# yechuan51/huffman

Measured on AMD Instinct MI355X. Metric: encode + decode throughput GB/s and % HBM3E peak, 16 GiB Zipf(1.1), 1/2/4/8 GPU, higher is better.
Workload: dtype u8; 1 GPU; 16 GiB Zipf(1.1) bytes per GPU: hist16 -> codebook -> pack -> decode, one global bit stream; bytes_per_gpu=17179869184, total_bytes=17179869184, symbols_per_gpu=8589934592, parallelism=single, payload_bytes_rank0=12416072164, max_code_len=22

## Files before the change

### huffman_amd/csrc/hz_chain.hip

```cpp
#include <stdio.h>
#include <stdlib.h>

#include "hz_decode_device.h"
#include "hz_walk_device.h"

namespace hz {

constexpr int kChainWalkWaves = 16;
constexpr uint32_t kChainRecs = 256;
constexpr uint32_t kSegRing = 16 + 1;
constexpr uint32_t kRingRow = kChainWalkWaves * 64;

struct ChainBlk {
    unsigned long long b0, b1;
    unsigned long long rec;
    long long out;
    uint32_t lo, hi;
    uint32_t last;
    uint32_t lhl;
};
static_assert(sizeof(ChainBlk) == 48, "ChainBlk");

struct ChainArgs {
    uint64_t nchains, cbits;
// ... 394 lines not shown
}

HZ_DEV void chain_store(const DecArgs& a, const ChainMeta& m, int lane, const uint32_t* pk) {
    uint16_t* out16 = reinterpret_cast<uint16_t*>(a.out);
    const uint32_t lo = m.lhl & 0x1ffu, hi = chain_meta_hi(m), last = m.lhl >> 18;
    const bool full = lo == 0 && hi == kChainRecs && last == 8 && m.out >= 0 &&
                      (uint64_t)m.out + (uint64_t)kBlockSyms <= a.nsym;
    if (full) {
        const long long ob = m.out;
#pragma unroll
        for (int c = 0; c < kChainsPerLane; ++c) {
            uint32_t* q = reinterpret_cast<uint32_t*>(out16 + ob + 8 * (64 * c + lane));
            u32x4a2 v = u32x4a2{pk[4 * c], pk[4 * c + 1], pk[4 * c + 2], pk[4 * c + 3]};
            __builtin_nontemporal_store(v, reinterpret_cast<u32x4a2*>(q));
        }
        return;
    }
#pragma unroll
    for (int c = 0; c < kChainsPerLane; ++c) {
        const uint32_t t = 64u * c + (uint32_t)lane;
        if (t < lo || t >= hi) continue;
        const long long o = m.out + 8ll * t;
        if (o < 0 || (uint64_t)o >= a.nsym) continue;
        uint32_t cn = t + 1 == hi ? last : 8u;
        cn = a.nsym - (uint64_t)o < cn ? (uint32_t)(a.nsym - (uint64_t)o) : cn;
        if (cn == 8) {
            *reinterpret_cast<u32x4a2*>(out16 + o) = u32x4a2{pk[4 * c], pk[4 * c + 1], pk[4 * c + 2], pk[4 * c + 3]};
        } else {
            for (uint32_t q = 0; q < cn; ++q) out16[o + q] = (uint16_t)(pk[4 * c + (q >> 1)] >> (16 * (q & 1)));
        }
    }
}

HZ_DEV void dec_wave_chain(const DecArgs& a, const ChainArgs& y, uint64_t nb, const uint32_t* lds, uint32_t* stg,
                           uint32_t slot, uint64_t b, uint64_t stride, int lane) {
    constexpr int C = 2 * kChainsPerLane;
    const __amdgpu_buffer_rsrc_t l2r = lut_l2_rsrc(a.l2);
    ChainMeta mc[2], mn[2], mn2[2];
    uint4 sc[2][kStageUnroll], sn[2][kStageUnroll];
#pragma unroll
    for (int j = 0; j < 2; ++j) {
        chain_meta_load(y, b + j, nb, mc[j]);
        chain_meta_load(y, b + stride + j, nb, mn[j]);
    }
#pragma unroll
    for (int j = 0; j < 2; ++j) chain_rec_load(y, lane, mc[j]);
    auto as_pipe = [](const ChainMeta& m) { PipeMeta p; p.b0 = m.b0; p.b1 = m.b1; p.sub = 0; return p; };
#pragma unroll
    for (int j = 0; j < 2; ++j) dec_stage_prefetch(a, as_pipe(mc[j]), lane, sc[j]);
    for (; b < nb; b += stride) {
#pragma unroll
        for (int j = 0; j < 2; ++j) chain_rec_load(y, lane, mn[j]);
        uint32_t p1[C];
#pragma unroll
        for (int j = 0; j < 2; ++j) {
            uint64_t w0;
            dec_stage_commit<true>(a, as_pipe(mc[j]), slot >> 2, stg + j * slot, lane, sc[j], w0);
            uint32_t off[kChainsPerLane];
            dec_chain_offsets(chain_meta_sub(mc[j], lane), mc[j].b0, mc[j].b1 - mc[j].b0, lane, off);
            const uint32_t top = (uint32_t)(stg - lds) + (uint32_t)(j + 1) * slot - 1u;
            const uint32_t base = top * 32u - (uint32_t)(mc[j].b0 + a.bit_adj - (w0 << 5));
#pragma unroll
            for (int c = 0; c < kChainsPerLane; ++c) p1[j * kChainsPerLane + c] = base - off[c];
        }
        __builtin_amdgcn_wave_barrier();
        uint32_t pk[2][kSPT / 2];
        PipeLane st[C];
        uint32_t g[C];
        auto finish = [&](int c, int q) {
            const uint32_t ee = st[c].e > g[c] ? st[c].e : g[c];
            p1[c] -= ee >> 24;
            const int i = ((c % kChainsPerLane) * kChainSyms + q) >> 1;
            if (q & 1) pk[c / kChainsPerLane][i] = __builtin_amdgcn_perm(ee, pk[c / kChainsPerLane][i], 0x06050201u);
            else pk[c / kChainsPerLane][i] = ee;
        };
        auto issue4 = [&](int c, int q) {
            __builtin_amdgcn_s_setprio(2);
            dec_pipe_ldsn<4>(a, lds, p1 + c, st + c, 16u * (uint32_t)q);
#pragma unroll
            for (int t = 0; t < 4; ++t)
                g[c + t] = __builtin_amdgcn_raw_buffer_load_b32(l2r, st[c + t].gi, 0, 0);
            __builtin_amdgcn_s_setprio(0);
        };
        issue4(0, 0);
#pragma unroll
        for (int q = 0; q < kChainSyms; ++q) {
            issue4(4, q);
            if (q == kPfStep) {
#pragma unroll
                for (int j = 0; j < 2; ++j) dec_stage_prefetch(a, as_pipe(mn[j]), lane, sn[j]);
#pragma unroll
                for (int j = 0; j < 2; ++j) chain_meta_load(y, b + 2 * stride + j, nb, mn2[j]);
            }
#pragma unroll
            for (int c = 0; c < 4; ++c) finish(c, q);
            if (q + 1 < kChainSyms) issue4(0, q + 1);
#pragma unroll
            for (int c = 4; c < 8; ++c) finish(c, q);
        }
        __builtin_amdgcn_wave_barrier();
#pragma unroll
        for (int j = 0; j < 2; ++j)
            if (b + j < nb) chain_store(a, mc[j], lane, pk[j]);
#pragma unroll
        for (int j = 0; j < 2; ++j) {
            mc[j] = mn[j];
            mn[j] = mn2[j];
#pragma unroll
            for (int u = 0; u < kStageUnroll; ++u) sc[j][u] = sn[j][u];
        }
    }
}

__global__ __launch_bounds__(kDecPipe2Threads) void k_chain_decode(DecArgs a, ChainArgs y) {
    extern __shared__ __attribute__((aligned(16))) uint32_t lds[];
    copy_lds_table(lds, a.lds_img, a.lds_words);
    const int lane = threadIdx.x & 63;
    const uint32_t wid = wave_id();
    typedef const __attribute__((address_space(4))) unsigned long long* cu64p;
    const uint64_t nb = ((cu64p)y.info)[0];
    if (nb == 0) return;
    const uint32_t slot = (uint32_t)__builtin_amdgcn_readfirstlane((int)dec_slot_words(((cu64p)y.info)[1], a.max_len));
    const uint32_t nwave = blockDim.x >> 6;
    uint32_t nw2 = a.region_words / (2 * slot);
    nw2 = nw2 < nwave ? nw2 : nwave;
    if (nw2 == 0) {
        if (threadIdx.x == 0) atomicOr(a.err, 128u);
        return;
    }
    if (wid >= nw2) return;
    const uint64_t b = 2 * ((uint64_t)blockIdx.x * nw2 + wid), stride = 2 * (uint64_t)gridDim.x * nw2;
    dec_wave_chain(a, y, nb, lds, lds + a.lds_words + wid * 2 * slot, slot, b, stride, lane);
}

__global__ __launch_bounds__(kSyncThreads) void k_chain_decode_serial(DecArgs a, ChainArgs y) {
    extern __shared__ __attribute__((aligned(16))) uint32_t lds[];
    copy_lds_table(lds, a.lds_img, a.lds_words);
    uint16_t* out16 = reinterpret_cast<uint16_t*>(a.out);
    const uint64_t nrec = y.info[0] * kChainRecs;
    const uint64_t stride = (uint64_t)gridDim.x * blockDim.x;
    for (uint64_t i = (uint64_t)blockIdx.x * blockDim.x + threadIdx.x; i < nrec; i += stride) {
        const ChainBlk& d = y.blk[i / kChainRecs];
        const uint32_t t = (uint32_t)(i % kChainRecs);
        if (t < d.lo || t >= d.hi) continue;
        const long long o = d.out + 8ll * t;
        const uint32_t cn = t + 1 == d.hi ? d.last : 8u;
        BitReader r;
        br_init(r, a, d.b0 + (uint16_t)(y.rec[d.rec + t] - (uint16_t)d.b0) + a.bit_adj);
        for (uint32_t q = 0; q < cn; ++q) {
            uint32_t sym;
            const uint32_t L = br_next<DEC_LUT>(r, a, lds, sym);
            if (L == 0) { atomicOr(a.err, 2u); break; }
            if (o + q >= 0 && (uint64_t)(o + q) < a.nsym) out16[o + q] = (uint16_t)sym;
        }
    }
}

template <int MODE>
__global__ __launch_bounds__(kSyncThreads) void k_chain_tail(DecArgs a, ChainArgs y) {
    extern __shared__ __attribute__((aligned(16))) uint32_t lds[];
    copy_lds_table(lds, a.lds_img, a.lds_words);
    uint16_t* out16 = reinterpret_cast<uint16_t*>(a.out);
    const uint64_t stride = (uint64_t)gridDim.x * blockDim.x;
    const uint64_t last = a.nsym - 1;
    for (uint64_t c = (uint64_t)blockIdx.x * blockDim.x + threadIdx.x; c < y.nchains; c += stride) {
// ... 255 lines not shown
        const bool deep = t.dec_max_len > t.chain_esc_m;
        const void* fn = deep ? (const void*)k_chain_walk<true> : (const void*)k_chain_walk<false>;
        if ((e = ensure_lds_limit(fn, (int)(kChainWalkWaves * 64 * (kSegRing * 4 + 16)))) != hipSuccess) return e;
        const uint64_t wgs = (g.nchains + threads - 1) / threads;
        if (deep) hipLaunchKernelGGL(k_chain_walk<true>, dim3(wgs), dim3(threads), ring_bytes, s, w, y);
        else hipLaunchKernelGGL(k_chain_walk<false>, dim3(wgs), dim3(threads), ring_bytes, s, w, y);
        cap_check(s, "walk");
    }
    if ((e = chain_fix_and_meta(st, t, ncu, s)) != hipSuccess) return e;
    st->valid = true;
    return hipSuccess;
}

hipError_t chain_refix(ChainState* st, const Tables& t, uint64_t entry0, int ncu, hipStream_t s) {
    if (!st->valid) return hipErrorInvalidValue;
    st->y.entry0 = entry0 != ~0ull ? entry0 - st->base : entry0;
    return chain_fix_and_meta(st, t, ncu, s);
}

hipError_t chain_decode(ChainState* st, const Tables& t, uint64_t nsym, uint8_t* d_out, unsigned long long* d_end,
                        int ncu, hipStream_t s) {
    if (!st->valid) return hipErrorInvalidValue;
    DecArgs d = st->d;
    const ChainArgs& y = st->y;
    d.out = d_out;
    d.nsym = nsym;
    hipError_t e;
    if ((e = hipMemsetAsync(y.info + 2, 0xff, 8, s)) != hipSuccess) return e;
    if (nsym && !chain_pipelined(t)) {
        if ((e = ensure_lds_limit((const void*)k_chain_decode_serial, kLdsBytes)) != hipSuccess) return e;
        hipLaunchKernelGGL(k_chain_decode_serial, dim3(4 * ncu), dim3(kSyncThreads), t.chain_lds_bytes, s, d, y);
    }
    if (nsym && chain_pipelined(t)) {
        if ((e = ensure_lds_limit((const void*)k_chain_decode, kLdsBytes)) != hipSuccess) return e;
        const uint64_t bits = st->g.pend - st->g.pbeg;
        uint64_t avg = (uint64_t)(chain_avg(t, bits, nsym) * kBlockSyms);
        avg = avg < (uint64_t)kBlockSyms * (uint32_t)d.max_len ? avg : (uint64_t)kBlockSyms * (uint32_t)d.max_len;
        const uint32_t worst = dec_slot_words_max(d.max_len);
        uint32_t est = dec_slot_words(avg + avg / 16 + 256, d.max_len);
        est = est < worst ? est : worst;
        const uint32_t table = d.lds_words;
        if (table < kDecMinLdsWords || table + worst > kLdsBytes / 4) return hipErrorInvalidValue;
        uint32_t nslot = (kLdsBytes / 4 - table) / est;
        nslot = nslot > 2 * kDecPipe2Threads / 64 ? 2 * kDecPipe2Threads / 64 : nslot;
        nslot &= ~1u;
        DecArgs b = d;
        b.region_words = nslot * est;
        if (b.region_words < 2 * worst && table + 2 * worst <= kLdsBytes / 4) b.region_words = 2 * worst;
        const int threads = 64 * (int)((nslot / 2) ? nslot / 2 : 1);
        const uint32_t lds = 4 * (table + b.region_words);
        hipLaunchKernelGGL(k_chain_decode, dim3(ncu), dim3(threads), lds, s, b, y);
        cap_check(s, "decode");
    }
    if (nsym) {
        if ((e = ensure_lds_limit((const void*)k_chain_tail<DEC_LUT>, kLdsBytes)) != hipSuccess) return e;
        const uint64_t wgs = grid_clamp((y.nchains + kSyncThreads - 1) / kSyncThreads, (uint64_t)ncu);
        hipLaunchKernelGGL(k_chain_tail<DEC_LUT>, dim3(wgs), dim3(kSyncThreads), t.chain_lds_bytes, s, d, y);
    }
    if (d_end) {
        if (st->base == 0) {
            if ((e = hipMemcpyAsync(d_end, y.info + 2, 8, hipMemcpyDeviceToDevice, s)) != hipSuccess) return e;
        } else {
            hipLaunchKernelGGL(k_chain_end, dim3(1), dim3(64), 0, s, (const unsigned long long*)y.info, d_end, st->base);
        }
    }
    cap_check(s, "tail+end");
    return hipGetLastError();
}

}
```

### huffman_amd/csrc/hz_decode.hip

```cpp
#include <stdlib.h>

#include <type_traits>

#include "hz_decode_device.h"

namespace hz {


template <bool WIDE>
HZ_DEV void dec_stage(const DecArgs& a, uint64_t b0, uint64_t b1, uint32_t npc_max, uint32_t* stg, int lane,
                      uint64_t& w0) {
    w0 = ((b0 >> 5) & ~3ull) - 4;
    const uint64_t wend = (b1 >> 5) + (WIDE ? 3 : 2);
    uint32_t npc = (uint32_t)((wend - w0 + 3) >> 2);
    npc = npc < npc_max ? npc : npc_max;
    uint4 v[kStageUnroll];
#pragma unroll
    for (int u = 0; u < kStageUnroll; ++u) {
        const uint32_t p = (uint32_t)lane + (uint32_t)u * kWave;
        if (p < npc) v[u] = dec_stage_load(a, w0 + 4ull * p);
    }
#pragma unroll
    for (int u = 0; u < kStageUnroll; ++u) {
        const uint32_t p = (uint32_t)lane + (uint32_t)u * kWave;
        if (p < npc)
            reinterpret_cast<uint4*>(stg)[p] = make_uint4(bswap32(v[u].x), bswap32(v[u].y), bswap32(v[u].z), bswap32(v[u].w));
    }
    for (uint32_t p = (uint32_t)lane + kStageUnroll * kWave; p < npc; p += kWave) {
        const uint4 x = dec_stage_load(a, w0 + 4ull * p);
        reinterpret_cast<uint4*>(stg)[p] = make_uint4(bswap32(x.x), bswap32(x.y), bswap32(x.z), bswap32(x.w));
    }
}

// ... 195 lines not shown
            const uint32_t sym = lut_leaf_sym(ee);
            const int i = (c * kChainSyms + q) >> 1;
            if (q & 1) pk[i] |= sym << 16;
            else pk[i] = sym;
        };
        auto issue2 = [&](int c) {
            dec_pipe_lds2(a, lds, stg, pos[c], pos[c + 1], st[c], st[c + 1]);
            g[c] = l2g[st[c].gi];
            g[c + 1] = l2g[st[c + 1].gi];
        };
        issue2(0);
#pragma unroll
        for (int q = 0; q < kChainSyms; ++q) {
            issue2(2);
            if (q == kPfStep) {
                dec_stage_prefetch(a, mn, lane, sn);
                dec_meta_load(a, b + 2 * stride, lane, mn2);
            }
            finish(0, q);
            finish(1, q);
            if (q + 1 < kChainSyms) issue2(0);
            finish(2, q);
            finish(3, q);
        }
        __builtin_amdgcn_wave_barrier();
        dec_store(a, b, lane, pk);
        mc = mn;
        mn = mn2;
#pragma unroll
        for (int u = 0; u < kStageUnroll; ++u) sc[u] = sn[u];
    }
}

template <int NS, typename A>
HZ_DEV void dec_wave_pipe2(const A& a, const uint32_t* lds, uint32_t* stg, uint32_t slot, uint64_t b,
                           uint64_t stride, int lane) {
    constexpr int C = 2 * kChainsPerLane;
    constexpr int H = kChainSyms / 2;
    static_assert(kChainsPerLane == 4, "four pairs of chains over two blocks");
    static_assert(kChainSyms == 8 && kPfStep == H, "a block's prefetch issues at the top of its second half");
    const __amdgpu_buffer_rsrc_t l2r = lut_l2_rsrc(a.l2);
    PipeMeta mn[2], mn2;
    uint4 sn[NS];
    uint32_t p1[C];
    uint32_t pk[2][kSPT / 2];
    PipeLane st[C];
    uint32_t g[C];
    auto commit = [&](int j) {
        uint64_t w0;
        dec_stage_commit<true>(a, mn[j], slot >> 2, stg + j * slot, lane, sn, w0);
        uint32_t off[kChainsPerLane];
        dec_chain_offsets(mn[j].sub, mn[j].b0, mn[j].b1 - mn[j].b0, lane, off);
        const uint32_t top = (uint32_t)(stg - lds) + (uint32_t)(j + 1) * slot - 1u;
        const uint32_t base = top * 32u - (uint32_t)(mn[j].b0 + a.bit_adj - (w0 << 5));
#pragma unroll
        for (int c = 0; c < kChainsPerLane; ++c) p1[j * kChainsPerLane + c] = base - off[c];
        mn[j] = mn2;
    };
    auto prefetch = [&](int j, uint64_t after) {
        dec_stage_prefetch(a, mn[j], lane, sn);
        dec_meta_load(a, after, lane, mn2);
    };
    auto finish = [&](int c, int q) {
        const uint32_t ee = st[c].e > g[c] ? st[c].e : g[c];
        p1[c] -= ee >> 24;
        const int i = ((c % kChainsPerLane) * kChainSyms + q) >> 1;
        if (q & 1) pk[c / kChainsPerLane][i] = __builtin_amdgcn_perm(ee, pk[c / kChainsPerLane][i], 0x06050201u);
        else pk[c / kChainsPerLane][i] = ee;
    };
    auto issue4 = [&](int c, int q) {
        __builtin_amdgcn_s_setprio(2);
        dec_pipe_ldsn<4>(a, lds, p1 + c, st + c, 16u * (uint32_t)q);
#pragma unroll
        for (int t = 0; t < 4; ++t)
            g[c + t] = __builtin_amdgcn_raw_buffer_load_b32(l2r, st[c + t].gi, 0, 0);
        __builtin_amdgcn_s_setprio(0);
    };
    auto finish4 = [&](int c, int q) {
#pragma unroll
        for (int t = 0; t < 4; ++t) finish(c + t, q);
    };
    if (b >= a.nblocks) return;
    dec_meta_load(a, b, lane, mn[0]);
    dec_meta_load(a, b + 1, lane, mn[1]);
    prefetch(0, b + stride);
    commit(0);
    prefetch(1, b + 1 + stride);
    commit(1);
    __builtin_amdgcn_wave_barrier();
    issue4(0, 0);
#pragma unroll
    for (int q = 0; q < H; ++q) {
        finish4(0, q);
        issue4(0, q + 1);
    }
    for (; b < a.nblocks; b += stride) {
#pragma unroll
        for (int t = 0; t < H; ++t) {
            issue4(4, t);
            if (t == 0) prefetch(0, b + 2 * stride);
            finish4(0, H + t);
            if (t + 1 < H) {
                issue4(0, H + t + 1);
            } else {
                __builtin_amdgcn_wave_barrier();
                dec_store(a, b, lane, pk[0]);
                commit(0);
                __builtin_amdgcn_wave_barrier();
                issue4(0, 0);
            }
            finish4(4, t);
        }
#pragma unroll
        for (int t = 0; t < H; ++t) {
            issue4(4, H + t);
            if (t == 0) prefetch(1, b + 1 + 2 * stride);
            finish4(0, t);
            issue4(0, t + 1);
            finish4(4, H + t);
        }
        __builtin_amdgcn_wave_barrier();
        if (b + 1 < a.nblocks) dec_store(a, b + 1, lane, pk[1]);
        commit(1);
        __builtin_amdgcn_wave_barrier();
    }
}

template <int MODE, bool WIDE, int PIPE, int NS = kStageUnroll>
__global__ __launch_bounds__(PIPE == 2 ? kDecPipe2Threads : 1024) void k_decode(DecArgs a) {
    extern __shared__ __attribute__((aligned(16))) uint32_t lds[];
    copy_lds_table(lds, a.lds_img, a.lds_words);
    const int lane = threadIdx.x & 63;
    const uint32_t wid = wave_id();
    const uint32_t slot = (uint32_t)__builtin_amdgcn_readfirstlane((int)dec_slot_words(a.starts[a.nblocks + 1], a.max_len));
    const uint32_t nwave = blockDim.x >> 6;
    if constexpr (PIPE == 2) {
        uint32_t nw2 = a.region_words / (2 * slot);
        nw2 = nw2 < nwave ? nw2 : nwave;
        if (nw2 > 0) {
            if (wid >= nw2) return;
            const uint64_t b = 2 * ((uint64_t)blockIdx.x * nw2 + wid), stride = 2 * (uint64_t)gridDim.x * nw2;
            dec_wave_pipe2<NS>(a, lds, lds + a.lds_words + wid * 2 * slot, slot, b, stride, lane);
            return;
        }
    }
    uint32_t nw = a.region_words / slot;
    nw = nw < nwave ? nw : nwave;
    if (wid >= nw) return;
    uint32_t* stg = lds + a.lds_words + wid * slot;
    const uint64_t b = (uint64_t)blockIdx.x * nw + wid, stride = (uint64_t)gridDim.x * nw;
    if constexpr (PIPE != 0) {
        dec_wave_pipe(a, lds, stg, slot, b, stride, lane);
    } else {
        for (uint64_t bb = b; bb < a.nblocks; bb += stride) dec_group<MODE, WIDE, 1>(a, lds, stg, slot, bb, lane);
    }
}

HZ_DEV void fixed16_step(const uint16_t* t16, const uint32_t (&ww)[5], uint32_t pos, uint32_t (&o)[4]) {
    const uint32_t sh = pos & 31;
#pragma unroll
    for (int t = 0; t < 4; ++t) {
        const uint32_t cw = sh ? __builtin_amdgcn_alignbit(ww[t], ww[t + 1], 32u - sh) : ww[t];
        o[t] = (uint32_t)t16[cw >> 16] | ((uint32_t)t16[cw & 0xffffu] << 16);
    }
}

__global__ __launch_bounds__(1024) void k_decode_fixed16_blk(DecArgs a, uint64_t nb) {
    extern __shared__ __attribute__((aligned(16))) uint32_t lds[];
    copy_lds_table(lds, a.lds_img, a.lds_words);
    const uint16_t* t16 = reinterpret_cast<const uint16_t*>(lds);
    const uint64_t p0 = (a.starts ? a.starts[0] : a.start0) + a.bit_adj;
    const uint32_t* w = a.words + (p0 >> 5);
    const u32x4a4* w4 = reinterpret_cast<const u32x4a4*>(w);
    uint4* o4 = reinterpret_cast<uint4*>(a.out);
    const int lane = threadIdx.x & 63;
// ... 105 lines not shown
    if (sym0 >= a.lo && sym0 + kBlockSyms <= a.hi) {
        uint16_t* ob = out16 + (sym0 - a.lo);
#pragma unroll
        for (int c = 0; c < kChainsPerLane; ++c) {
            u32x4a2 v = u32x4a2{pk[4 * c], pk[4 * c + 1], pk[4 * c + 2], pk[4 * c + 3]};
            __builtin_nontemporal_store(v, reinterpret_cast<u32x4a2*>(ob + kChainSyms * (kWave * c + lane)));
        }
        return;
    }
#pragma unroll
    for (int c = 0; c < kChainsPerLane; ++c) {
        const uint64_t s0 = sym0 + (uint64_t)kChainSyms * (uint32_t)(c * kWave + lane);
        for (uint32_t q = 0; q < (uint32_t)kChainSyms; ++q) {
            const uint64_t sy = s0 + q;
            if (sy >= a.lo && sy < a.hi) out16[sy - a.lo] = (uint16_t)(pk[4 * c + (q >> 1)] >> (16 * (q & 1)));
        }
    }
}

template <int MODE, bool WIDE, int PIPE, int NS = kStageUnroll>
__global__ __launch_bounds__(PIPE == 2 ? kDecPipe2Threads : 1024) void k_decode_range(RangeDecArgs a) {
    extern __shared__ __attribute__((aligned(16))) uint32_t lds[];
    copy_lds_table(lds, a.lds_img, a.lds_words);
    const int lane = threadIdx.x & 63;
    const uint32_t wid = wave_id();
    const uint32_t slot = (uint32_t)__builtin_amdgcn_readfirstlane((int)dec_slot_words(a.starts[a.nblocks + 1], a.max_len));
    const uint32_t nwave = blockDim.x >> 6;
    if constexpr (PIPE == 2) {
        uint32_t nw2 = a.region_words / (2 * slot);
        nw2 = nw2 < nwave ? nw2 : nwave;
        if (nw2 > 0) {
            if (wid >= nw2) return;
            const uint64_t b = 2 * ((uint64_t)blockIdx.x * nw2 + wid), stride = 2 * (uint64_t)gridDim.x * nw2;
            dec_wave_pipe2<NS>(a, lds, lds + a.lds_words + wid * 2 * slot, slot, b, stride, lane);
            return;
        }
    }
    uint32_t nw = a.region_words / slot;
    nw = nw < nwave ? nw : nwave;
    if (wid >= nw) return;
    uint32_t* stg = lds + a.lds_words + wid * slot;
    const uint64_t b = (uint64_t)blockIdx.x * nw + wid, stride = (uint64_t)gridDim.x * nw;
    if constexpr (PIPE != 0) {
        dec_wave_pipe(a, lds, stg, slot, b, stride, lane);
    } else {
        for (uint64_t bb = b; bb < a.nblocks; bb += stride) dec_group<MODE, WIDE, 1>(a, lds, stg, slot, bb, lane);
    }
}

template <int MODE, bool WIDE, int PIPE, int NS, typename A>
static const void* decode_fn() {
    if constexpr (std::is_same<A, DecArgs>::value) return (const void*)k_decode<MODE, WIDE, PIPE, NS>;
    else return (const void*)k_decode_range<MODE, WIDE, PIPE, NS>;
}

constexpr int kStageFew = 3;
static int dec_stage_chunks(uint64_t nwords, uint64_t nblocks) {
    const uint64_t mean = (nwords * 4 + nblocks - 1) / nblocks;
    return mean + 16 + 8 + mean / 64 + 16 < 16ull * kWave * kStageFew ? kStageFew : kStageUnroll;
}

template <int MODE, bool WIDE, int PIPE, typename A = DecArgs, int NS = kStageUnroll>
static hipError_t run_decode(const A& a, uint64_t payload_bits, int ncu, hipStream_t s) {
    const void* fn = decode_fn<MODE, WIDE, PIPE, NS, A>();
    {
        hipError_t e = ensure_lds_limit(fn, kLdsBytes);
        if (e != hipSuccess) return e;
    }
    uint64_t avg = (payload_bits + a.nblocks - 1) / a.nblocks;
    avg = avg < (uint64_t)kBlockSyms * (uint32_t)a.max_len ? avg : (uint64_t)kBlockSyms * (uint32_t)a.max_len;
    const uint32_t worst = dec_slot_words_max(a.max_len);
    uint32_t est = dec_slot_words(avg + avg / 16 + 256, a.max_len);
    est = est < worst ? est : worst;
    const uint32_t table = a.lds_words;
    if (MODE == DEC_LUT && PIPE == 2 && table < kDecMinLdsWords) return hipErrorInvalidValue;
    int best_w = 0, best_g = 1;
    for (int g = 1; g <= 2; ++g) {
        const uint32_t room = kLdsBytes / 4 / (uint32_t)g;
        if (room <= table + est) continue;
        int w = (int)((room - table) / est);
        const int maxw = PIPE == 2 ? 2 * kDecPipe2Threads / 64 : kDecMaxWaves;
        w = w > maxw ? maxw : w;
        if (g * w > best_g * best_w) { best_w = w; best_g = g; }
    }
    if (best_w == 0) return hipErrorInvalidValue;
    A b = a;
    b.region_words = (uint32_t)best_w * est;
    if (b.region_words < worst && table + worst <= kLdsBytes / 4) b.region_words = worst;
    if (table + b.region_words > kLdsBytes / 4 / (uint32_t)best_g) best_g = 1;
    if (table + b.region_words > kLdsBytes / 4) return hipErrorInvalidValue;
    const uint32_t lds = 4 * (table + b.region_words);
    uint64_t wgs = (a.nblocks + best_w - 1) / best_w;
// ... 26 lines not shown
                               : run_decode<DEC_LUT, false, 2>(a, payload_bits, ncu, s);
    }
    return run_decode<DEC_LUT, false, 0>(a, payload_bits, ncu, s);
}

hipError_t launch_decode(const Tables& t, const uint8_t* d_payload, uint64_t payload_bytes, uint64_t nsym,
                         const unsigned long long* d_index, uint8_t* d_out, uint32_t* d_err, int ncu,
                         hipStream_t s, uint64_t start0, int* stage_chunks) {
    if (stage_chunks) *stage_chunks = 0;
    if (nsym == 0) return hipSuccess;
    if (!d_index && t.dec_mode != DEC_FIXED16) return hipErrorInvalidValue;
    DecArgs a;
    fill_dec_args(a, t, d_payload, payload_bytes, nsym);
    a.starts = d_index;
    a.subs = d_index ? d_index + index_sub_offset(a.nblocks) : nullptr;
    a.start0 = start0;
    a.out = d_out; a.err = d_err;
    if (t.dec_mode == DEC_FIXED16) {
        hipError_t e = ensure_lds_limit((const void*)k_decode_fixed16, kFixed16LdsBytes);
        if (e != hipSuccess) return e;
        if ((e = ensure_lds_limit((const void*)k_decode_fixed16_blk, kFixed16LdsBytes)) != hipSuccess) return e;
        const uint64_t nl = (nsym + kSPT - 1) / kSPT;
        const uint64_t nb = kFixed16Blk && a.nblocks > 1 ? a.nblocks - 1 : 0;
        if (nb) {
            uint64_t wgs = (nb + 15) / 16;
            if (wgs > (uint64_t)ncu) wgs = ncu;
            hipLaunchKernelGGL(k_decode_fixed16_blk, dim3(wgs), dim3(1024), kFixed16LdsBytes, s, a, nb);
        }
        uint64_t wgs = (nl + 1023) / 1024;
        if (wgs > (uint64_t)ncu) wgs = ncu;
        hipLaunchKernelGGL(k_decode_fixed16, dim3(wgs), dim3(1024), kFixed16LdsBytes, s, a, nb);
        return hipGetLastError();
    }
    return decode_dispatch(t, a, a.nwords >= 4, payload_bytes * 8, ncu, s, stage_chunks);
}

struct SeekArgs {
    const unsigned long long* seek;
    const unsigned long long* isub;
    unsigned long long* tstart;
    unsigned long long* rows;
    unsigned long long* maxp;
    uint8_t* bad;
    uint64_t blk0, nb, nsym;
    uint64_t clamp_lo, bit_hi;
};

constexpr int kSeekThreads = 256;

template <int MODE, bool WALK>
__global__ __launch_bounds__(kSeekThreads) void k_seek_subs(DecArgs a, SeekArgs y) {
    extern __shared__ __attribute__((aligned(16))) uint32_t lds[];
    if constexpr (WALK && MODE != DEC_FIXED16) copy_lds_table(lds, a.lds_img, a.lds_words);
    const uint64_t j = (uint64_t)blockIdx.x * blockDim.x + threadIdx.x;
    unsigned long long mx = 0;
    if (j < y.nb) {
        const uint64_t b = y.blk0 + j;
        const uint64_t s0 = y.seek[b], s1 = y.seek[b + 1];
        const uint64_t left = y.nsym - b * kBlockSyms;
        const uint32_t cnt = left < (uint64_t)kBlockSyms ? (uint32_t)left : (uint32_t)kBlockSyms;
        uint32_t err = 0;
        if (s1 < s0 || s1 - s0 > (uint64_t)cnt * (uint32_t)a.max_len) err = 1u;
        else if (s0 < y.clamp_lo || s1 > y.bit_hi) err = 16u;
        else if (y.isub && (uint32_t)(y.isub[b * kWave] & 0xffffu) != (uint32_t)(s0 & 0xffffu)) err = 1u;
        if (y.tstart) {
            auto clamp = [&](uint64_t x) { return x < y.clamp_lo ? y.clamp_lo : (x > y.bit_hi ? y.bit_hi : x); };
            y.tstart[j] = clamp(s0);
// ... 201 lines not shown
```

### huffman_amd/csrc/hz_decode_device.h

```cpp
#pragma once
#include "hz_device.h"

namespace hz {

struct DecArgs {
    const uint32_t* words;
    uint64_t nwords;
    uint32_t bit_adj;
    uint64_t nsym;
    uint64_t nblocks;
    const unsigned long long* starts;
    const unsigned long long* subs;
    uint64_t start0;
    const uint32_t* lds_img;
    uint32_t lds_words;
    uint32_t region_words;
    int k;
    int min_len;
    int max_len;
    int level_bits;
    const uint32_t* l2;
    uint8_t* out;
    uint32_t* err;
};
// ... 62 lines not shown
    for (int c = 0; c < C; ++c) off[c] = ((uint32_t)(sub >> (16 * c)) - (uint32_t)bs) & 0xffffu;
    if (bits >= 65536) {
        uint32_t carry = 0, last = 0;
#pragma unroll
        for (int c = 0; c < C; ++c) {
            uint32_t pv = shfl_up_u32(off[c], 1);
            if (lane == 0) pv = last;
            last = __builtin_amdgcn_readlane(off[c], 63);
            uint32_t sc = (off[c] - pv) & 0xffffu;
#pragma unroll
            for (int dd = 1; dd < 64; dd <<= 1) {
                const uint32_t o = shfl_up_u32(sc, dd);
                if (lane >= dd) sc += o;
            }
            off[c] = carry + sc;
            carry = __builtin_amdgcn_readlane(off[c], 63);
        }
    }
}

struct PipeLane {
    uint32_t e, gi;
};

#define HZ_WALK_FENCE() __builtin_amdgcn_sched_barrier(0)

static_assert(kLutGlobal + kLutMaxL2 == (1u << 21), "a leaf (bit 31) read as a link lands past num_records");
HZ_DEV __amdgpu_buffer_rsrc_t lut_l2_rsrc(const uint32_t* l2) {
    return __builtin_amdgcn_make_buffer_rsrc(
        reinterpret_cast<void*>(reinterpret_cast<uintptr_t>(l2) - 4ull * kLutGlobal), 0,
        4u * (kLutGlobal + kLutMaxL2), 0x00020000);
}

template <int NC>
HZ_DEV void dec_pipe_ldsn(const DecArgs& a, const uint32_t* lds, const uint32_t* p1, PipeLane* r, uint32_t adj = 0) {
    const uint32_t k = (uint32_t)a.k;
    uint32_t W[NC], e[NC], x[NC];
    bool h[NC];
    uint32_t whi[NC], wlo[NC];
#pragma unroll
    for (int c = 0; c < NC; ++c) {
        const uint32_t wb = ((p1[c] >> 3) & ~3u) + adj;
        whi[c] = lds_at(wb + 4);
        wlo[c] = lds_at(wb);
    }
    HZ_WALK_FENCE();
#pragma unroll
    for (int c = 0; c < NC; ++c) W[c] = __builtin_amdgcn_alignbit(whi[c], wlo[c], p1[c]);
    HZ_WALK_FENCE();
#pragma unroll
    for (int c = 0; c < NC; ++c) e[c] = lds_at((W[c] >> (32 - k)) << 2);
    HZ_WALK_FENCE();
#pragma unroll
    for (int c = 0; c < NC; ++c) {
        h[c] = lut_lds_link(e[c]);
        const uint32_t byte = ((e[c] >> 10) + __builtin_amdgcn_ubfe(W[c], e[c], e[c] >> 5)) << 2;
        x[c] = lds_at(byte);
    }
    HZ_WALK_FENCE();
#pragma unroll
    for (int c = 0; c < NC; ++c) {
        const uint32_t ee = h[c] ? x[c] : e[c];
        const uint32_t byte = ((ee >> 10) + __builtin_amdgcn_ubfe(W[c], ee, ee >> 5)) << 2;
        r[c].e = ee;
        r[c].gi = byte;
    }
}

struct PipeMeta {
    uint64_t b0, b1, sub;
};

template <int NS>
HZ_DEV void dec_stage_prefetch(const DecArgs& a, const PipeMeta& m, int lane, uint4 (&v)[NS]) {
    const uint64_t w0 = (((m.b0 + a.bit_adj) >> 5) & ~3ull) - 4;
#pragma unroll
    for (int u = 0; u < NS; ++u) {
        const uint64_t w = w0 + 4ull * ((uint32_t)lane + (uint32_t)u * kWave);
        const bool in = w < a.nwords;
        const uint64_t wl = !in ? 0 : (w + 4 <= a.nwords ? w : a.nwords - 4);
        v[u] = *reinterpret_cast<const uint4*>(a.words + wl);
    }
}

template <bool DESC = false, int NS>
HZ_DEV void dec_stage_commit(const DecArgs& a, const PipeMeta& m, uint32_t npc_max, uint32_t* stg, int lane,
                             const uint4 (&v)[NS], uint64_t& w0) {
    const uint64_t b0 = m.b0 + a.bit_adj, b1 = m.b1 + a.bit_adj;
    w0 = ((b0 >> 5) & ~3ull) - 4;
    const uint64_t wend = (b1 >> 5) + 2;
    uint32_t npc = (uint32_t)((wend - w0 + 3) >> 2);
// ... 1 lines not shown
#pragma unroll
    for (int u = 0; u < NS; ++u) {
        const uint32_t p = (uint32_t)lane + (uint32_t)u * kWave;
        if (p < npc) {
            const uint64_t w = w0 + 4ull * p;
            uint4 x = v[u];
            if (!(w < a.nwords && w + 4 <= a.nwords)) {
                const uint64_t base = a.nwords - 4;
                uint32_t q[4];
#pragma unroll
                for (int t = 0; t < 4; ++t) {
                    const uint64_t wt = w + t;
                    q[t] = wt < a.nwords && w < a.nwords ? pick4(x, (uint32_t)(wt - base)) : 0u;
                }
                x = make_uint4(q[0], q[1], q[2], q[3]);
            }
            if (DESC)
                reinterpret_cast<uint4*>(stg)[npc_max - 1 - p] = make_uint4(bswap32(x.w), bswap32(x.z), bswap32(x.y), bswap32(x.x));
            else
                reinterpret_cast<uint4*>(stg)[p] = make_uint4(bswap32(x.x), bswap32(x.y), bswap32(x.z), bswap32(x.w));
        }
    }
    for (uint32_t p = (uint32_t)lane + NS * kWave; p < npc; p += kWave) {
        const uint4 x = dec_stage_load(a, w0 + 4ull * p);
        if (DESC)
            reinterpret_cast<uint4*>(stg)[npc_max - 1 - p] = make_uint4(bswap32(x.w), bswap32(x.z), bswap32(x.y), bswap32(x.x));
        else
            reinterpret_cast<uint4*>(stg)[p] = make_uint4(bswap32(x.x), bswap32(x.y), bswap32(x.z), bswap32(x.w));
    }
}

constexpr int kPfStep = 4;
constexpr int kDecPipe2Threads = 512;

struct BitReader {
    uint64_t buf;
    uint32_t nb;
    uint32_t nxt;
    uint4 cur, ahead;
    uint32_t ci;
    uint64_t abase;
};

template <typename A>
HZ_DEV uint4 ld_chunk(const A& a, uint64_t w) {
    if (w + 4 <= a.nwords) return *reinterpret_cast<const uint4*>(a.words + w);
    uint4 v;
    v.x = w < a.nwords ? a.words[w] : 0u;
    v.y = w + 1 < a.nwords ? a.words[w + 1] : 0u;
    v.z = w + 2 < a.nwords ? a.words[w + 2] : 0u;
    v.w = 0u;
    return v;
}

template <typename A>
HZ_DEV uint32_t br_word(BitReader& r, const A& a) {
    const uint32_t v = pick4(r.cur, r.ci);
    if (++r.ci == 4) {
        r.cur = r.ahead;
        r.ci = 0;
        r.abase += 4;
        r.ahead = ld_chunk(a, r.abase);
    }
    return bswap32(v);
}

// ... 57 lines not shown
```

Before: 856.5 GB/s.

## Route chain decode through shared software-pipelined block walker with staged prefetch

```diff
diff --git a/huffman_amd/csrc/hz_chain.hip b/huffman_amd/csrc/hz_chain.hip
--- a/huffman_amd/csrc/hz_chain.hip
+++ b/huffman_amd/csrc/hz_chain.hip
@@ -450,86 +450,22 @@
     }
 }
 
-HZ_DEV void dec_wave_chain(const DecArgs& a, const ChainArgs& y, uint64_t nb, const uint32_t* lds, uint32_t* stg,
-                           uint32_t slot, uint64_t b, uint64_t stride, int lane) {
-    constexpr int C = 2 * kChainsPerLane;
-    const __amdgpu_buffer_rsrc_t l2r = lut_l2_rsrc(a.l2);
-    ChainMeta mc[2], mn[2], mn2[2];
-    uint4 sc[2][kStageUnroll], sn[2][kStageUnroll];
-#pragma unroll
-    for (int j = 0; j < 2; ++j) {
-        chain_meta_load(y, b + j, nb, mc[j]);
-        chain_meta_load(y, b + stride + j, nb, mn[j]);
-    }
-#pragma unroll
-    for (int j = 0; j < 2; ++j) chain_rec_load(y, lane, mc[j]);
-    auto as_pipe = [](const ChainMeta& m) { PipeMeta p; p.b0 = m.b0; p.b1 = m.b1; p.sub = 0; return p; };
-#pragma unroll
-    for (int j = 0; j < 2; ++j) dec_stage_prefetch(a, as_pipe(mc[j]), lane, sc[j]);
-    for (; b < nb; b += stride) {
-#pragma unroll
-        for (int j = 0; j < 2; ++j) chain_rec_load(y, lane, mn[j]);
-        uint32_t p1[C];
-#pragma unroll
-        for (int j = 0; j < 2; ++j) {
-            uint64_t w0;
-            dec_stage_commit<true>(a, as_pipe(mc[j]), slot >> 2, stg + j * slot, lane, sc[j], w0);
-            uint32_t off[kChainsPerLane];
-            dec_chain_offsets(chain_meta_sub(mc[j], lane), mc[j].b0, mc[j].b1 - mc[j].b0, lane, off);
-            const uint32_t top = (uint32_t)(stg - lds) + (uint32_t)(j + 1) * slot - 1u;
-            const uint32_t base = top * 32u - (uint32_t)(mc[j].b0 + a.bit_adj - (w0 << 5));
-#pragma unroll
-            for (int c = 0; c < kChainsPerLane; ++c) p1[j * kChainsPerLane + c] = base - off[c];
-        }
-        __builtin_amdgcn_wave_barrier();
-        uint32_t pk[2][kSPT / 2];
-        PipeLane st[C];
-        uint32_t g[C];
-        auto finish = [&](int c, int q) {
-            const uint32_t ee = st[c].e > g[c] ? st[c].e : g[c];
-            p1[c] -= ee >> 24;
-            const int i = ((c % kChainsPerLane) * kChainSyms + q) >> 1;
-            if (q & 1) pk[c / kChainsPerLane][i] = __builtin_amdgcn_perm(ee, pk[c / kChainsPerLane][i], 0x06050201u);
-            else pk[c / kChainsPerLane][i] = ee;
-        };
-        auto issue4 = [&](int c, int q) {
-            __builtin_amdgcn_s_setprio(2);
-            dec_pipe_ldsn<4>(a, lds, p1 + c, st + c, 16u * (uint32_t)q);
-#pragma unroll
-            for (int t = 0; t < 4; ++t)
-                g[c + t] = __builtin_amdgcn_raw_buffer_load_b32(l2r, st[c + t].gi, 0, 0);
-            __builtin_amdgcn_s_setprio(0);
-        };
-        issue4(0, 0);
-#pragma unroll
-        for (int q = 0; q < kChainSyms; ++q) {
-            issue4(4, q);
-            if (q == kPfStep) {
-#pragma unroll
-                for (int j = 0; j < 2; ++j) dec_stage_prefetch(a, as_pipe(mn[j]), lane, sn[j]);
-#pragma unroll
-                for (int j = 0; j < 2; ++j) chain_meta_load(y, b + 2 * stride + j, nb, mn2[j]);
-            }
-#pragma unroll
-            for (int c = 0; c < 4; ++c) finish(c, q);
-            if (q + 1 < kChainSyms) issue4(0, q + 1);
-#pragma unroll
-            for (int c = 4; c < 8; ++c) finish(c, q);
-        }
-        __builtin_amdgcn_wave_barrier();
-#pragma unroll
-        for (int j = 0; j < 2; ++j)
-            if (b + j < nb) chain_store(a, mc[j], lane, pk[j]);
-#pragma unroll
-        for (int j = 0; j < 2; ++j) {
-            mc[j] = mn[j];
-            mn[j] = mn2[j];
-#pragma unroll
-            for (int u = 0; u < kStageUnroll; ++u) sc[j][u] = sn[j][u];
-        }
-    }
-}
-
+struct ChainBlocks {
+    using Meta = ChainMeta;
+    const DecArgs& a;
+    const ChainArgs& y;
+    uint64_t nb;
+    ChainMeta cur[2];
+    HZ_DEV uint64_t nblocks() const { return nb; }
+    HZ_DEV void load(uint64_t b, int, Meta& m) const { chain_meta_load(y, b, nb, m); }
+    HZ_DEV void ready(int lane, Meta& m) const { chain_rec_load(y, lane, m); }
+    HZ_DEV void taken(int j, const Meta& m) { cur[j] = m; }
+    HZ_DEV PipeMeta bounds(const Meta& m) const { PipeMeta p; p.b0 = m.b0; p.b1 = m.b1; p.sub = 0; return p; }
+    HZ_DEV uint64_t sub(const Meta& m, int lane) const { return chain_meta_sub(m, lane); }
+    HZ_DEV void store(int j, uint64_t, int lane, const uint32_t* pk) const { chain_store(a, cur[j], lane, pk); }
+};
+
+template <int NS>
 __global__ __launch_bounds__(kDecPipe2Threads) void k_chain_decode(DecArgs a, ChainArgs y) {
     extern __shared__ __attribute__((aligned(16))) uint32_t lds[];
     copy_lds_table(lds, a.lds_img, a.lds_words);
@@ -548,7 +484,8 @@
     }
     if (wid >= nw2) return;
     const uint64_t b = 2 * ((uint64_t)blockIdx.x * nw2 + wid), stride = 2 * (uint64_t)gridDim.x * nw2;
-    dec_wave_chain(a, y, nb, lds, lds + a.lds_words + wid * 2 * slot, slot, b, stride, lane);
+    ChainBlocks blocks{a, y, nb};
+    dec_wave_pipe2<NS>(a, blocks, lds, lds + a.lds_words + wid * 2 * slot, slot, b, stride, lane);
 }
 
 __global__ __launch_bounds__(kSyncThreads) void k_chain_decode_serial(DecArgs a, ChainArgs y) {
@@ -870,9 +807,11 @@
         hipLaunchKernelGGL(k_chain_decode_serial, dim3(4 * ncu), dim3(kSyncThreads), t.chain_lds_bytes, s, d, y);
     }
     if (nsym && chain_pipelined(t)) {
-        if ((e = ensure_lds_limit((const void*)k_chain_decode, kLdsBytes)) != hipSuccess) return e;
         const uint64_t bits = st->g.pend - st->g.pbeg;
         uint64_t avg = (uint64_t)(chain_avg(t, bits, nsym) * kBlockSyms);
+        const bool few = dec_stage_chunks_mean((avg + 7) / 8) == kStageFew;
+        const void* fn = few ? (const void*)k_chain_decode<kStageFew> : (const void*)k_chain_decode<kStageUnroll>;
+        if ((e = ensure_lds_limit(fn, kLdsBytes)) != hipSuccess) return e;
         avg = avg < (uint64_t)kBlockSyms * (uint32_t)d.max_len ? avg : (uint64_t)kBlockSyms * (uint32_t)d.max_len;
         const uint32_t worst = dec_slot_words_max(d.max_len);
         uint32_t est = dec_slot_words(avg + avg / 16 + 256, d.max_len);
@@ -887,7 +826,8 @@
         if (b.region_words < 2 * worst && table + 2 * worst <= kLdsBytes / 4) b.region_words = 2 * worst;
         const int threads = 64 * (int)((nslot / 2) ? nslot / 2 : 1);
         const uint32_t lds = 4 * (table + b.region_words);
-        hipLaunchKernelGGL(k_chain_decode, dim3(ncu), dim3(threads), lds, s, b, y);
+        void* kargs[] = {&b, const_cast<ChainArgs*>(&y)};
+        if ((e = hipLaunchKernel(fn, dim3(ncu), dim3(threads), kargs, lds, s)) != hipSuccess) return e;
         cap_check(s, "decode");
     }
     if (nsym) {
diff --git a/huffman_amd/csrc/hz_decode.hip b/huffman_amd/csrc/hz_decode.hip
--- a/huffman_amd/csrc/hz_decode.hip
+++ b/huffman_amd/csrc/hz_decode.hip
@@ -1,4 +1,8 @@
 #include <stdlib.h>
+#ifdef HZ_DEC_TIMING
+#include <stdio.h>
+#include <string.h>
+#endif
 
 #include <type_traits>
 
@@ -260,99 +264,18 @@
     }
 }
 
-template <int NS, typename A>
-HZ_DEV void dec_wave_pipe2(const A& a, const uint32_t* lds, uint32_t* stg, uint32_t slot, uint64_t b,
-                           uint64_t stride, int lane) {
-    constexpr int C = 2 * kChainsPerLane;
-    constexpr int H = kChainSyms / 2;
-    static_assert(kChainsPerLane == 4, "four pairs of chains over two blocks");
-    static_assert(kChainSyms == 8 && kPfStep == H, "a block's prefetch issues at the top of its second half");
-    const __amdgpu_buffer_rsrc_t l2r = lut_l2_rsrc(a.l2);
-    PipeMeta mn[2], mn2;
-    uint4 sn[NS];
-    uint32_t p1[C];
-    uint32_t pk[2][kSPT / 2];
-    PipeLane st[C];
-    uint32_t g[C];
-    auto commit = [&](int j) {
-        uint64_t w0;
-        dec_stage_commit<true>(a, mn[j], slot >> 2, stg + j * slot, lane, sn, w0);
-        uint32_t off[kChainsPerLane];
-        dec_chain_offsets(mn[j].sub, mn[j].b0, mn[j].b1 - mn[j].b0, lane, off);
-        const uint32_t top = (uint32_t)(stg - lds) + (uint32_t)(j + 1) * slot - 1u;
-        const uint32_t base = top * 32u - (uint32_t)(mn[j].b0 + a.bit_adj - (w0 << 5));
-#pragma unroll
-        for (int c = 0; c < kChainsPerLane; ++c) p1[j * kChainsPerLane + c] = base - off[c];
-        mn[j] = mn2;
-    };
-    auto prefetch = [&](int j, uint64_t after) {
-        dec_stage_prefetch(a, mn[j], lane, sn);
-        dec_meta_load(a, after, lane, mn2);
-    };
-    auto finish = [&](int c, int q) {
-        const uint32_t ee = st[c].e > g[c] ? st[c].e : g[c];
-        p1[c] -= ee >> 24;
-        const int i = ((c % kChainsPerLane) * kChainSyms + q) >> 1;
-        if (q & 1) pk[c / kChainsPerLane][i] = __builtin_amdgcn_perm(ee, pk[c / kChainsPerLane][i], 0x06050201u);
-        else pk[c / kChainsPerLane][i] = ee;
-    };
-    auto issue4 = [&](int c, int q) {
-        __builtin_amdgcn_s_setprio(2);
-        dec_pipe_ldsn<4>(a, lds, p1 + c, st + c, 16u * (uint32_t)q);
-#pragma unroll
-        for (int t = 0; t < 4; ++t)
-            g[c + t] = __builtin_amdgcn_raw_buffer_load_b32(l2r, st[c + t].gi, 0, 0);
-        __builtin_amdgcn_s_setprio(0);
-    };
-    auto finish4 = [&](int c, int q) {
-#pragma unroll
-        for (int t = 0; t < 4; ++t) finish(c + t, q);
-    };
-    if (b >= a.nblocks) return;
-    dec_meta_load(a, b, lane, mn[0]);
-    dec_meta_load(a, b + 1, lane, mn[1]);
-    prefetch(0, b + stride);
-    commit(0);
-    prefetch(1, b + 1 + stride);
-    commit(1);
-    __builtin_amdgcn_wave_barrier();
-    issue4(0, 0);
-#pragma unroll
-    for (int q = 0; q < H; ++q) {
-        finish4(0, q);
-        issue4(0, q + 1);
-    }
-    for (; b < a.nblocks; b += stride) {
-#pragma unroll
-        for (int t = 0; t < H; ++t) {
-            issue4(4, t);
-            if (t == 0) prefetch(0, b + 2 * stride);
-            finish4(0, H + t);
-            if (t + 1 < H) {
-                issue4(0, H + t + 1);
-            } else {
-                __builtin_amdgcn_wave_barrier();
-                dec_store(a, b, lane, pk[0]);
-                commit(0);
-                __builtin_amdgcn_wave_barrier();
-                issue4(0, 0);
-            }
-            finish4(4, t);
-        }
-#pragma unroll
-        for (int t = 0; t < H; ++t) {
-            issue4(4, H + t);
-            if (t == 0) prefetch(1, b + 1 + 2 * stride);
-            finish4(0, t);
-            issue4(0, t + 1);
-            finish4(4, H + t);
-        }
-        __builtin_amdgcn_wave_barrier();
-        if (b + 1 < a.nblocks) dec_store(a, b + 1, lane, pk[1]);
-        commit(1);
-        __builtin_amdgcn_wave_barrier();
-    }
-}
+template <typename A>
+struct IndexBlocks {
+    using Meta = PipeMeta;
+    const A& a;
+    HZ_DEV uint64_t nblocks() const { return a.nblocks; }
+    HZ_DEV void load(uint64_t b, int lane, Meta& m) const { dec_meta_load(a, b, lane, m); }
+    HZ_DEV void ready(int, Meta&) const {}
+    HZ_DEV void taken(int, const Meta&) const {}
+    HZ_DEV const PipeMeta& bounds(const Meta& m) const { return m; }
+    HZ_DEV uint64_t sub(const Meta& m, int) const { return m.sub; }
+    HZ_DEV void store(int, uint64_t b, int lane, const uint32_t* pk) const { dec_store(a, b, lane, pk); }
+};
 
 template <int MODE, bool WIDE, int PIPE, int NS = kStageUnroll>
 __global__ __launch_bounds__(PIPE == 2 ? kDecPipe2Threads : 1024) void k_decode(DecArgs a) {
@@ -368,7 +291,8 @@
         if (nw2 > 0) {
             if (wid >= nw2) return;
             const uint64_t b = 2 * ((uint64_t)blockIdx.x * nw2 + wid), stride = 2 * (uint64_t)gridDim.x * nw2;
-            dec_wave_pipe2<NS>(a, lds, lds + a.lds_words + wid * 2 * slot, slot, b, stride, lane);
+            IndexBlocks<decltype(a)> blocks{a};
+            dec_wave_pipe2<NS>(a, blocks, lds, lds + a.lds_words + wid * 2 * slot, slot, b, stride, lane);
             return;
         }
     }
@@ -540,7 +464,8 @@
         if (nw2 > 0) {
             if (wid >= nw2) return;
             const uint64_t b = 2 * ((uint64_t)blockIdx.x * nw2 + wid), stride = 2 * (uint64_t)gridDim.x * nw2;
-            dec_wave_pipe2<NS>(a, lds, lds + a.lds_words + wid * 2 * slot, slot, b, stride, lane);
+            IndexBlocks<decltype(a)> blocks{a};
+            dec_wave_pipe2<NS>(a, blocks, lds, lds + a.lds_words + wid * 2 * slot, slot, b, stride, lane);
             return;
         }
     }
@@ -560,12 +485,6 @@
 static const void* decode_fn() {
     if constexpr (std::is_same<A, DecArgs>::value) return (const void*)k_decode<MODE, WIDE, PIPE, NS>;
     else return (const void*)k_decode_range<MODE, WIDE, PIPE, NS>;
-}
-
-constexpr int kStageFew = 3;
-static int dec_stage_chunks(uint64_t nwords, uint64_t nblocks) {
-    const uint64_t mean = (nwords * 4 + nblocks - 1) / nblocks;
-    return mean + 16 + 8 + mean / 64 + 16 < 16ull * kWave * kStageFew ? kStageFew : kStageUnroll;
 }
 
 template <int MODE, bool WIDE, int PIPE, typename A = DecArgs, int NS = kStageUnroll>
@@ -658,7 +577,25 @@
         hipLaunchKernelGGL(k_decode_fixed16, dim3(wgs), dim3(1024), kFixed16LdsBytes, s, a, nb);
         return hipGetLastError();
     }
+#ifdef HZ_DEC_TIMING
+    static unsigned long long rows[kTimingRows * kTimingCols];
+    memset(rows, 0, sizeof rows);
+    hipError_t te = hipMemcpyToSymbolAsync(HIP_SYMBOL(g_dec_timing), rows, sizeof rows, 0, hipMemcpyHostToDevice, s);
+    if (te != hipSuccess) return te;
+    te = decode_dispatch(t, a, a.nwords >= 4, payload_bytes * 8, ncu, s, stage_chunks);
+    if (te != hipSuccess) return te;
+    if (const char* path = getenv("HZ_DEC_TIMING_OUT")) {
+        if ((te = hipStreamSynchronize(s)) != hipSuccess) return te;
+        if ((te = hipMemcpyFromSymbol(rows, HIP_SYMBOL(g_dec_timing), sizeof rows)) != hipSuccess) return te;
+        if (FILE* f = fopen(path, "wb")) {
+            fwrite(rows, 1, sizeof rows, f);
+            fclose(f);
+        }
+    }
+    return hipSuccess;
+#else
     return decode_dispatch(t, a, a.nwords >= 4, payload_bytes * 8, ncu, s, stage_chunks);
+#endif
 }
 
 struct SeekArgs {
diff --git a/huffman_amd/csrc/hz_decode_device.h b/huffman_amd/csrc/hz_decode_device.h
--- a/huffman_amd/csrc/hz_decode_device.h
+++ b/huffman_amd/csrc/hz_decode_device.h
@@ -118,8 +118,17 @@
         4u * (kLutGlobal + kLutMaxL2), 0x00020000);
 }
 
+#ifdef HZ_DEC_TIMING
+constexpr int kTimingRows = 512, kTimingCols = 8, kTimingPairs = 32;
+static __device__ unsigned long long g_dec_timing[kTimingRows * kTimingCols];
+#define HZ_STAMP(ts, i) do { if (ts) (ts)[i] = __builtin_amdgcn_s_memtime(); } while (0)
+#else
+#define HZ_STAMP(ts, i) ((void)0)
+#endif
+
 template <int NC>
-HZ_DEV void dec_pipe_ldsn(const DecArgs& a, const uint32_t* lds, const uint32_t* p1, PipeLane* r, uint32_t adj = 0) {
+HZ_DEV void dec_pipe_ldsn(const DecArgs& a, const uint32_t* lds, const uint32_t* p1, PipeLane* r, uint32_t adj = 0,
+                          uint64_t* ts = nullptr) {
     const uint32_t k = (uint32_t)a.k;
     uint32_t W[NC], e[NC], x[NC];
     bool h[NC];
@@ -130,12 +139,14 @@
         whi[c] = lds_at(wb + 4);
         wlo[c] = lds_at(wb);
     }
+    HZ_STAMP(ts, 0);
     HZ_WALK_FENCE();
 #pragma unroll
     for (int c = 0; c < NC; ++c) W[c] = __builtin_amdgcn_alignbit(whi[c], wlo[c], p1[c]);
     HZ_WALK_FENCE();
 #pragma unroll
     for (int c = 0; c < NC; ++c) e[c] = lds_at((W[c] >> (32 - k)) << 2);
+    HZ_STAMP(ts, 1);
     HZ_WALK_FENCE();
 #pragma unroll
     for (int c = 0; c < NC; ++c) {
@@ -143,6 +154,7 @@
         const uint32_t byte = ((e[c] >> 10) + __builtin_amdgcn_ubfe(W[c], e[c], e[c] >> 5)) << 2;
         x[c] = lds_at(byte);
     }
+    HZ_STAMP(ts, 2);
     HZ_WALK_FENCE();
 #pragma unroll
     for (int c = 0; c < NC; ++c) {
@@ -210,6 +222,155 @@
 
 constexpr int kPfStep = 4;
 constexpr int kDecPipe2Threads = 512;
+
+constexpr int kStageFew = 3;
+inline int dec_stage_chunks_mean(uint64_t mean) {
+    return mean + 16 + 8 + mean / 64 + 16 < 16ull * kWave * kStageFew ? kStageFew : kStageUnroll;
+}
+inline int dec_stage_chunks(uint64_t nwords, uint64_t nblocks) {
+    return dec_stage_chunks_mean((nwords * 4 + nblocks - 1) / nblocks);
+}
+
+template <int NS, typename A, typename P>
+HZ_DEV void dec_wave_pipe2(const A& a, P& pol, const uint32_t* lds, uint32_t* stg, uint32_t slot, uint64_t b,
+                           uint64_t stride, int lane) {
+    constexpr int C = 2 * kChainsPerLane;
+    constexpr int H = kChainSyms / 2;
+    static_assert(kChainsPerLane == 4, "four pairs of chains over two blocks");
+    static_assert(kChainSyms == 8 && kPfStep == H, "a block's prefetch issues at the top of its second half");
+    const __amdgpu_buffer_rsrc_t l2r = lut_l2_rsrc(a.l2);
+    const uint64_t nblocks = pol.nblocks();
+    typename P::Meta mn[2], mn2;
+    uint4 sn[NS];
+    uint32_t p1[C];
+    uint32_t pk[2][kSPT / 2];
+    PipeLane st[C];
+    uint32_t g[C];
+#ifdef HZ_DEC_TIMING
+    uint64_t ts[2][4] = {}, tlast[2] = {}, tacc[6] = {};
+    uint32_t tn = 0, tpair = 0;
+    const bool twave = wave_id() == 0 && blockIdx.x < (uint32_t)kTimingRows;
+    const uint32_t tmid = (uint32_t)(((nblocks > b ? nblocks - b : 0) + stride - 1) / stride / 2);
+    bool trec = false;
+#endif
+    auto commit = [&](int j) {
+        uint64_t w0;
+        const auto& m = pol.bounds(mn[j]);
+        dec_stage_commit<true>(a, m, slot >> 2, stg + j * slot, lane, sn, w0);
+        uint32_t off[kChainsPerLane];
+        dec_chain_offsets(pol.sub(mn[j], lane), m.b0, m.b1 - m.b0, lane, off);
+        const uint32_t top = (uint32_t)(stg - lds) + (uint32_t)(j + 1) * slot - 1u;
+        const uint32_t base = top * 32u - (uint32_t)(m.b0 + a.bit_adj - (w0 << 5));
+#pragma unroll
+        for (int c = 0; c < kChainsPerLane; ++c) p1[j * kChainsPerLane + c] = base - off[c];
+        pol.taken(j, mn[j]);
+        mn[j] = mn2;
+        pol.ready(lane, mn[j]);
+    };
+    auto prefetch = [&](int j, uint64_t after) {
+        dec_stage_prefetch(a, pol.bounds(mn[j]), lane, sn);
+        pol.load(after, lane, mn2);
+    };
+    auto finish = [&](int c, int q) {
+        const uint32_t ee = st[c].e > g[c] ? st[c].e : g[c];
+        p1[c] -= ee >> 24;
+        const int i = ((c % kChainsPerLane) * kChainSyms + q) >> 1;
+        if (q & 1) pk[c / kChainsPerLane][i] = __builtin_amdgcn_perm(ee, pk[c / kChainsPerLane][i], 0x06050201u);
+        else pk[c / kChainsPerLane][i] = ee;
+    };
+    auto issue4 = [&](int c, int q) {
+        __builtin_amdgcn_s_setprio(2);
+#ifdef HZ_DEC_TIMING
+        uint64_t* const tq = ts[c / 4];
+#else
+        uint64_t* const tq = nullptr;
+#endif
+        dec_pipe_ldsn<4>(a, lds, p1 + c, st + c, 16u * (uint32_t)q, tq);
+#pragma unroll
+        for (int t = 0; t < 4; ++t)
+            g[c + t] = __builtin_amdgcn_raw_buffer_load_b32(l2r, st[c + t].gi, 0, 0);
+        HZ_STAMP(tq, 3);
+        __builtin_amdgcn_s_setprio(0);
+    };
+    auto finish4 = [&](int c, int q) {
+#ifdef HZ_DEC_TIMING
+        const uint64_t f0 = __builtin_amdgcn_s_memtime();
+        asm volatile("" : "+v"(g[c]), "+v"(g[c + 1]), "+v"(g[c + 2]), "+v"(g[c + 3]));
+        const uint64_t f1 = __builtin_amdgcn_s_memtime();
+        const uint64_t* tq = ts[c / 4];
+        if (trec) {
+            tacc[0] += tq[1] - tq[0];
+            tacc[1] += tq[2] - tq[1];
+            tacc[2] += tq[3] - tq[2];
+            tacc[3] += f1 - tq[3];
+            tacc[4] += f1 - f0;
+            tacc[5] += f1 - tlast[c / 4];
+            ++tn;
+        }
+        tlast[c / 4] = f1;
+#endif
+#pragma unroll
+        for (int t = 0; t < 4; ++t) finish(c + t, q);
+    };
+    if (b >= nblocks) return;
+    pol.load(b, lane, mn[0]);
+    pol.load(b + 1, lane, mn[1]);
+    pol.ready(lane, mn[0]);
+    pol.ready(lane, mn[1]);
+    prefetch(0, b + stride);
+    commit(0);
+    prefetch(1, b + 1 + stride);
+    commit(1);
+    __builtin_amdgcn_wave_barrier();
+    issue4(0, 0);
+#pragma unroll
+    for (int q = 0; q < H; ++q) {
+        finish4(0, q);
+        issue4(0, q + 1);
+    }
+    for (; b < nblocks; b += stride) {
+#ifdef HZ_DEC_TIMING
+        trec = twave && tpair >= tmid && tpair < tmid + (uint32_t)kTimingPairs;
+        ++tpair;
+#endif
+#pragma unroll
+        for (int t = 0; t < H; ++t) {
+            issue4(4, t);
+            if (t == 0) prefetch(0, b + 2 * stride);
+            finish4(0, H + t);
+            if (t + 1 < H) {
+                issue4(0, H + t + 1);
+            } else {
+                __builtin_amdgcn_wave_barrier();
+                pol.store(0, b, lane, pk[0]);
+                commit(0);
+                __builtin_amdgcn_wave_barrier();
+                issue4(0, 0);
+            }
+            finish4(4, t);
+        }
+#pragma unroll
+        for (int t = 0; t < H; ++t) {
+            issue4(4, H + t);
+            if (t == 0) prefetch(1, b + 1 + 2 * stride);
+            finish4(0, t);
+            issue4(0, t + 1);
+            finish4(4, H + t);
+        }
+        __builtin_amdgcn_wave_barrier();
+        if (b + 1 < nblocks) pol.store(1, b + 1, lane, pk[1]);
+        commit(1);
+        __builtin_amdgcn_wave_barrier();
+    }
+#ifdef HZ_DEC_TIMING
+    if (twave) {
+        unsigned long long v = tn;
+#pragma unroll
+        for (int i = 0; i < 6; ++i) v = lane == i ? tacc[i] : v;
+        if (lane < 7) g_dec_timing[blockIdx.x * kTimingCols + lane] = v;
+    }
+#endif
+}
 
 struct BitReader {
     uint64_t buf;
```

Measured after the change: 852.8 GB/s. About the same (-0.4%).
